# markvdw/GParML

Measured on AMD Instinct MI355X. Metric: variational bound+grad evals/sec, higher is better.
Workload: dtype f64

## Files before the change

gparml_amd/csrc/potrf128.h:

```cpp
#pragma once
#include <hip/hip_runtime.h>
#include "mma_f64.h"

#ifndef POTRF_STAMP
#define POTRF_STAMP(i)
#endif

namespace gp {

constexpr int NB = 128;

constexpr int PLD = NB + 2;

__device__ __forceinline__ void wave_sync() {
  asm volatile("s_waitcnt lgkmcnt(0)" ::: "memory");
  __builtin_amdgcn_wave_barrier();
}
__device__ __forceinline__ void block_sync_lds() {
  asm volatile("s_waitcnt lgkmcnt(0)" ::: "memory");
  __builtin_amdgcn_s_barrier();
  asm volatile("" ::: "memory");
}

__device__ __forceinline__ double readlane_f64(double v, int src) {
  const int lo = __builtin_amdgcn_readlane(__double2loint(v), src), hi = __builtin_amdgcn_readlane(__double2hiint(v), src);
  return __hiloint2double(hi, lo);
}

__device__ __forceinline__ double rsqrt_chain(double x) {
  const double y = __builtin_amdgcn_rsq(x);
  const double e = fma(-(x * y), y, 1.0);
  return fma(y * e, fma(e, 0.375, 0.5), y);
}

template <bool BT>
__device__ __forceinline__ void lds_mma16(const double* S, int ar, int ac, int br, int bc, int kb, int ke, int lane, double (&acc)[4]) {
  const int lr = lane & 15, lk = lane >> 4, lj = lane & 3;
  const double* pa = S + (ar + lr) * PLD + ac + lk;
  const double* pb = BT ? S + (br + lj) * PLD + bc + lk : S + (br + lk) * PLD + bc + lj;
  auto load = [&](int k0, double (&a)[4], double (&b)[4][4]) {
#pragma unroll
    for (int s = 0; s < 4; ++s) {
      const int k = k0 + 4 * s;
      a[s] = pa[k];
#pragma unroll
      for (int j = 0; j < 4; ++j) b[s][j] = BT ? pb[4 * j * PLD + k] : pb[k * PLD + 4 * j];
    }
  };
  auto mma = [&](const double (&a)[4], const double (&b)[4][4]) {
    __builtin_amdgcn_sched_barrier(0);
#pragma unroll
    for (int s = 0; s < 4; ++s)
#pragma unroll
      for (int j = 0; j < 4; ++j) acc[j] = __builtin_amdgcn_mfma_f64_4x4x4f64(a[s], b[s][j], acc[j], 0, 0, 0);
    __builtin_amdgcn_sched_barrier(0);
  };
  double a0[4], b0[4][4], a1[4], b1[4][4];
  if (kb < ke) load(kb, a0, b0);
  for (int k = kb; k < ke; k += 32) {
    const bool more1 = k + 16 < ke, more2 = k + 32 < ke;
    if (more1) load(k + 16, a1, b1);
    mma(a0, b0);
    if (more1) {
      if (more2) load(k + 32, a0, b0);
      mma(a1, b1);
    }
  }
}
__device__ __forceinline__ int t16_row(int lane) { return 4 * ((lane >> 2) & 3) + (lane >> 4); }
__device__ __forceinline__ int t16_col(int j, int lane) { return 4 * j + (lane & 3); }

constexpr int LSLD = 34;
constexpr int POTRF_LDS_DOUBLES = NB * PLD + 32 + 32 * LSLD + NB;

__global__ void __launch_bounds__(512) potrf_trinv128_kernel(double* A, long ld, long bstride, int j, double* Linv, double* fail,
                                                             double* logdet2) {
  extern __shared__ __attribute__((aligned(16))) double sm[];
  double* S = sm;
  double* Tw = S + NB * PLD;
  double* Lsp = Tw + 32;
  double* Dg = Lsp + 32 * LSLD;
  const int tid = threadIdx.x, lane = tid & 63, wave = __builtin_amdgcn_readfirstlane(tid >> 6);
  const long off = (long)blockIdx.x * bstride + ((long)j * NB) * ld + (long)j * NB;
  double* blk = A + off;
  double* xblk = Linv + off;
  {
    double2 v[16];
#pragma unroll
    for (int i = 0; i < 16; ++i) { const int e = tid + 512 * i; v[i] = *reinterpret_cast<const double2*>(blk + (long)(e >> 6) * ld + 2 * (e & 63)); }
#pragma unroll
    for (int i = 0; i < 16; ++i) {
      const int e = tid + 512 * i, r = e >> 6, c = 2 * (e & 63);
      *reinterpret_cast<double2*>(S + r * PLD + c) = make_double2(c <= r ? v[i].x : 0.0, c + 1 <= r ? v[i].y : 0.0);
    }
  }
  __syncthreads();
  POTRF_STAMP(0);
  double bad = 0.0;
  for (int s = 0; s < 4; ++s) {
    const int o = 32 * s;
    if (wave == 0) {
      const int i = lane & 31;
      double a[32];
#pragma unroll
      for (int p = 0; p < 16; ++p) {
        const double2 v = *reinterpret_cast<const double2*>(S + (o + i) * PLD + o + 2 * p);
        a[2 * p] = v.x; a[2 * p + 1] = v.y;
      }
      double myinv = 1.0, mydiag = 1.0;
      static_for<0, 32>([&](auto jc) {
        constexpr int j = decltype(jc)::value;
        const double d = readlane_f64(a[j], j);
        if (!(d > 0.0)) bad = fmax(bad, d == 0.0 ? 2.0 : 1.0);
        const double inv = rsqrt_chain(d);
        const double l = a[j] * inv;
        a[j] = l;
        if (i == j) { myinv = inv; mydiag = l; }
        static_for<j + 1, 32>([&](auto kc) {
          constexpr int k = decltype(kc)::value;
          a[k] = fma(-l, readlane_f64(l, k), a[k]);
        });
      });
      POTRF_STAMP(1 + 5 * s);
      if (lane < 32) {
#pragma unroll
        for (int p = 0; p < 16; ++p) {
          const double2 v = make_double2(2 * p <= i ? a[2 * p] : 0.0, 2 * p + 1 <= i ? a[2 * p + 1] : 0.0);
          *reinterpret_cast<double2*>(S + (o + i) * PLD + o + 2 * p) = v;
          *reinterpret_cast<double2*>(Lsp + i * LSLD + 2 * p) = v;
        }
        Tw[i] = myinv;
        Dg[o + i] = mydiag;
      }
      wave_sync();
      POTRF_STAMP(2 + 5 * s);
      if (lane < 32) {
        const int h = lane >> 4, cl = lane & 15;
        double w[16];
        double2 row[2][8];
        double dinv[2];
        const double* Ls = S + (o + 16 * h) * PLD + o + 16 * h;
        const double* Tl = Tw + 16 * h;
        auto load_row = [&](auto ic, double2 (&b)[8], double& d) {
          constexpr int i = decltype(ic)::value;
#pragma unroll
          for (int p = 0; p < (i + 1) / 2; ++p) b[p] = *reinterpret_cast<const double2*>(Ls + i * PLD + 2 * p);
          d = Tl[i];
        };
        load_row(IC<0>{}, row[0], dinv[0]);
        static_for<0, 16>([&](auto ic) {
          constexpr int i = decltype(ic)::value, cur = i & 1;
          if constexpr (i + 1 < 16) load_row(IC<i + 1>{}, row[cur ^ 1], dinv[cur ^ 1]);
          __builtin_amdgcn_sched_barrier(0);
          double s0 = (cl == i) ? 1.0 : 0.0, s1 = 0.0;
#pragma unroll
          for (int p = 0; p < i / 2; ++p) {
            s0 = fma(-row[cur][p].x, w[2 * p], s0);
            s1 = fma(-row[cur][p].y, w[2 * p + 1], s1);
          }
          if constexpr (i & 1) s0 = fma(-row[cur][i / 2].x, w[i - 1], s0);
          w[i] = (s0 + s1) * dinv[cur];
          __builtin_amdgcn_sched_barrier(0);
        });
#pragma unroll
        for (int i = 0; i < 16; ++i) S[(o + 16 * h + i) * PLD + o + 16 * h + cl] = w[i];
      }
      wave_sync();
      {
        double acc[4] = {0.0, 0.0, 0.0, 0.0};
        lds_mma16<false>(S, o + 16, o, o, o, 0, 16, lane, acc);
        wave_sync();
        const int R = o + 16 + t16_row(lane);
#pragma unroll
        for (int jj = 0; jj < 4; ++jj) { S[R * PLD + o + t16_col(jj, lane)] = acc[jj]; acc[jj] = 0.0; }
        wave_sync();
        lds_mma16<false>(S, o + 16, o + 16, o + 16, o, 0, 16, lane, acc);
        wave_sync();
#pragma unroll
        for (int jj = 0; jj < 4; ++jj) S[R * PLD + o + t16_col(jj, lane)] = -acc[jj];
      }
      wave_sync();
    }
    block_sync_lds();
    POTRF_STAMP(3 + 5 * s);
    if (wave == 7) {
#pragma unroll
      for (int it = 0; it < 8; ++it) {
        const int e = lane + 64 * it, r = e >> 4, c = 2 * (e & 15);
        *reinterpret_cast<double2*>(blk + (long)(o + r) * ld + o + c) = *reinterpret_cast<const double2*>(Lsp + r * LSLD + c);
      }
    }
    if (s == 3) break;
    const int nrb = (NB - o - 32) / 16;
    {
      double acc[2][4] = {{0.0, 0.0, 0.0, 0.0}, {0.0, 0.0, 0.0, 0.0}};
#pragma unroll
      for (int u = 0; u < 2; ++u) {
        const int t = wave + 8 * u;
        if (t < 2 * nrb) lds_mma16<true>(S, o + 32 + 16 * (t >> 1), o, o + 16 * (t & 1), o, 0, 16 * (t & 1) + 16, lane, acc[u]);
      }
      block_sync_lds();
#pragma unroll
      for (int u = 0; u < 2; ++u) {
        const int t = wave + 8 * u;
        if (t < 2 * nrb) {
          const int R = o + 32 + 16 * (t >> 1) + t16_row(lane);
#pragma unroll
          for (int jj = 0; jj < 4; ++jj) {
            const int C = o + 16 * (t & 1) + t16_col(jj, lane);
            S[R * PLD + C] = acc[u][jj];
            blk[(long)R * ld + C] = acc[u][jj];
          }
        }
      }
      block_sync_lds();
    }
    POTRF_STAMP(4 + 5 * s);
    auto update_tile = [&](int t) {
      int r16 = 0, rem = t;
      while (rem > r16) { rem -= r16 + 1; ++r16; }
      const int c16 = rem;
      double acc[4] = {0.0, 0.0, 0.0, 0.0};
      lds_mma16<true>(S, o + 32 + 16 * r16, o, o + 32 + 16 * c16, o, 0, 32, lane, acc);
      const int R = o + 32 + 16 * r16 + t16_row(lane);
#pragma unroll
      for (int jj = 0; jj < 4; ++jj) S[R * PLD + o + 32 + 16 * c16 + t16_col(jj, lane)] -= acc[jj];
    };
    const int ntile = nrb * (nrb + 1) / 2;
    if (wave < ntile) update_tile(wave);
    block_sync_lds();
    if (wave > 0)
      for (int t = 8 + (wave - 1); t < ntile; t += 7) update_tile(t);
    POTRF_STAMP(5 + 5 * s);
  }
  auto level = [&](auto bsc) {
    constexpr int bs = decltype(bsc)::value, tpp = (bs / 16) * (bs / 16), ntask = (NB / (2 * bs)) * tpp;
    double acc[2][4] = {{0.0, 0.0, 0.0, 0.0}, {0.0, 0.0, 0.0, 0.0}};
    int R0[2], C0[2], rb[2], cb[2];
#pragma unroll
    for (int u = 0; u < 2; ++u) {
      const int t = wave + 8 * u, p = t / tpp, tt = t % tpp;
      R0[u] = (2 * p + 1) * bs; C0[u] = 2 * p * bs; rb[u] = tt / (bs / 16); cb[u] = tt % (bs / 16);
      if (t < ntask) lds_mma16<false>(S, R0[u] + 16 * rb[u], C0[u], C0[u], C0[u] + 16 * cb[u], 16 * cb[u], bs, lane, acc[u]);
    }
    block_sync_lds();
#pragma unroll
    for (int u = 0; u < 2; ++u) {
      if (wave + 8 * u < ntask) {
        const int R = R0[u] + 16 * rb[u] + t16_row(lane);
#pragma unroll
        for (int jj = 0; jj < 4; ++jj) { S[R * PLD + C0[u] + 16 * cb[u] + t16_col(jj, lane)] = acc[u][jj]; acc[u][jj] = 0.0; }
      }
    }
    block_sync_lds();
#pragma unroll
    for (int u = 0; u < 2; ++u)
      if (wave + 8 * u < ntask) lds_mma16<false>(S, R0[u] + 16 * rb[u], R0[u], R0[u], C0[u] + 16 * cb[u], 0, 16 * rb[u] + 16, lane, acc[u]);
    block_sync_lds();
#pragma unroll
    for (int u = 0; u < 2; ++u) {
      if (wave + 8 * u < ntask) {
        const int R = R0[u] + 16 * rb[u] + t16_row(lane);
#pragma unroll
        for (int jj = 0; jj < 4; ++jj) S[R * PLD + C0[u] + 16 * cb[u] + t16_col(jj, lane)] = -acc[u][jj];
      }
    }
    block_sync_lds();
  };
  level(IC<32>{});
  level(IC<64>{});
  POTRF_STAMP(20);
  {
    int t2 = tid;
    asm volatile("" : "+v"(t2));
#pragma unroll
    for (int i = 0; i < 16; ++i) {
      const int e = t2 + 512 * i, r = e >> 6, c = 2 * (e & 63);
      const double2 x = *reinterpret_cast<const double2*>(S + r * PLD + c);
      *reinterpret_cast<double2*>(xblk + (long)r * ld + c) = make_double2(c <= r ? x.x : 0.0, c + 1 <= r ? x.y : 0.0);
      if (c > r) *reinterpret_cast<double2*>(blk + (long)r * ld + c) = make_double2(0.0, 0.0);
      else if (c == r) blk[(long)r * ld + c + 1] = 0.0;
    }
  }
  POTRF_STAMP(21);
  if (wave == 0) {
    double lg = log(Dg[lane]) + log(Dg[lane + 64]);
    for (int sh = 32; sh > 0; sh >>= 1) { lg += __shfl_xor(lg, sh); bad = fmax(bad, __shfl_xor(bad, sh)); }
    if (lane == 0) {
      if (bad != 0.0) fail[blockIdx.x] = fmax(fail[blockIdx.x], bad);
      logdet2[blockIdx.x] += 2.0 * lg;
    }
  }
}

}
```

Baseline: 57.48.

## Shrink Cholesky panel width to 16 and overlap diagonal factorization with trailing update

```diff
diff --git a/gparml_amd/csrc/potrf128.h b/gparml_amd/csrc/potrf128.h
--- a/gparml_amd/csrc/potrf128.h
+++ b/gparml_amd/csrc/potrf128.h
@@ -70,16 +70,17 @@
 __device__ __forceinline__ int t16_row(int lane) { return 4 * ((lane >> 2) & 3) + (lane >> 4); }
 __device__ __forceinline__ int t16_col(int j, int lane) { return 4 * j + (lane & 3); }
 
-constexpr int LSLD = 34;
-constexpr int POTRF_LDS_DOUBLES = NB * PLD + 32 + 32 * LSLD + NB;
+constexpr int SB = 16;
+constexpr int LSLD = 18;
+constexpr int POTRF_LDS_DOUBLES = NB * PLD + SB + 2 * SB * LSLD + NB;
 
 __global__ void __launch_bounds__(512) potrf_trinv128_kernel(double* A, long ld, long bstride, int j, double* Linv, double* fail,
                                                              double* logdet2) {
   extern __shared__ __attribute__((aligned(16))) double sm[];
   double* S = sm;
   double* Tw = S + NB * PLD;
-  double* Lsp = Tw + 32;
-  double* Dg = Lsp + 32 * LSLD;
+  double* Lsp = Tw + SB;
+  double* Dg = Lsp + 2 * SB * LSLD;
   const int tid = threadIdx.x, lane = tid & 63, wave = __builtin_amdgcn_readfirstlane(tid >> 6);
   const long off = (long)blockIdx.x * bstride + ((long)j * NB) * ld + (long)j * NB;
   double* blk = A + off;
@@ -97,18 +98,18 @@
   __syncthreads();
   POTRF_STAMP(0);
   double bad = 0.0;
-  for (int s = 0; s < 4; ++s) {
-    const int o = 32 * s;
+  for (int s = 0; s < NB / SB; ++s) {
+    const int o = SB * s;
     if (wave == 0) {
-      const int i = lane & 31;
-      double a[32];
-#pragma unroll
-      for (int p = 0; p < 16; ++p) {
+      const int i = lane & (SB - 1);
+      double a[SB];
+#pragma unroll
+      for (int p = 0; p < SB / 2; ++p) {
         const double2 v = *reinterpret_cast<const double2*>(S + (o + i) * PLD + o + 2 * p);
         a[2 * p] = v.x; a[2 * p + 1] = v.y;
       }
       double myinv = 1.0, mydiag = 1.0;
-      static_for<0, 32>([&](auto jc) {
+      static_for<0, SB>([&](auto jc) {
         constexpr int j = decltype(jc)::value;
         const double d = readlane_f64(a[j], j);
         if (!(d > 0.0)) bad = fmax(bad, d == 0.0 ? 2.0 : 1.0);
@@ -116,31 +117,31 @@
         const double l = a[j] * inv;
         a[j] = l;
         if (i == j) { myinv = inv; mydiag = l; }
-        static_for<j + 1, 32>([&](auto kc) {
+        static_for<j + 1, SB>([&](auto kc) {
           constexpr int k = decltype(kc)::value;
           a[k] = fma(-l, readlane_f64(l, k), a[k]);
         });
       });
-      POTRF_STAMP(1 + 5 * s);
-      if (lane < 32) {
-#pragma unroll
-        for (int p = 0; p < 16; ++p) {
+      POTRF_STAMP(1 + 4 * s);
+      double* Lcopy = Lsp + (s & 1) * SB * LSLD;
+      if (lane < SB) {
+#pragma unroll
+        for (int p = 0; p < SB / 2; ++p) {
           const double2 v = make_double2(2 * p <= i ? a[2 * p] : 0.0, 2 * p + 1 <= i ? a[2 * p + 1] : 0.0);
           *reinterpret_cast<double2*>(S + (o + i) * PLD + o + 2 * p) = v;
-          *reinterpret_cast<double2*>(Lsp + i * LSLD + 2 * p) = v;
+          *reinterpret_cast<double2*>(Lcopy + i * LSLD + 2 * p) = v;
         }
         Tw[i] = myinv;
         Dg[o + i] = mydiag;
       }
       wave_sync();
-      POTRF_STAMP(2 + 5 * s);
-      if (lane < 32) {
-        const int h = lane >> 4, cl = lane & 15;
+      if (lane < SB) {
+        const int cl = lane;
         double w[16];
         double2 row[2][8];
         double dinv[2];
-        const double* Ls = S + (o + 16 * h) * PLD + o + 16 * h;
-        const double* Tl = Tw + 16 * h;
+        const double* Ls = S + o * PLD + o;
+        const double* Tl = Tw;
         auto load_row = [&](auto ic, double2 (&b)[8], double& d) {
           constexpr int i = decltype(ic)::value;
 #pragma unroll
@@ -163,75 +164,54 @@
           __builtin_amdgcn_sched_barrier(0);
         });
 #pragma unroll
-        for (int i = 0; i < 16; ++i) S[(o + 16 * h + i) * PLD + o + 16 * h + cl] = w[i];
-      }
-      wave_sync();
-      {
-        double acc[4] = {0.0, 0.0, 0.0, 0.0};
-        lds_mma16<false>(S, o + 16, o, o, o, 0, 16, lane, acc);
-        wave_sync();
-        const int R = o + 16 + t16_row(lane);
-#pragma unroll
-        for (int jj = 0; jj < 4; ++jj) { S[R * PLD + o + t16_col(jj, lane)] = acc[jj]; acc[jj] = 0.0; }
-        wave_sync();
-        lds_mma16<false>(S, o + 16, o + 16, o + 16, o, 0, 16, lane, acc);
-        wave_sync();
-#pragma unroll
-        for (int jj = 0; jj < 4; ++jj) S[R * PLD + o + t16_col(jj, lane)] = -acc[jj];
-      }
-      wave_sync();
-    }
-    block_sync_lds();
-    POTRF_STAMP(3 + 5 * s);
+        for (int i = 0; i < 16; ++i) S[(o + i) * PLD + o + cl] = w[i];
+      }
+      wave_sync();
+      POTRF_STAMP(2 + 4 * s);
+    }
+    block_sync_lds();
     if (wave == 7) {
-#pragma unroll
-      for (int it = 0; it < 8; ++it) {
-        const int e = lane + 64 * it, r = e >> 4, c = 2 * (e & 15);
-        *reinterpret_cast<double2*>(blk + (long)(o + r) * ld + o + c) = *reinterpret_cast<const double2*>(Lsp + r * LSLD + c);
-      }
-    }
-    if (s == 3) break;
-    const int nrb = (NB - o - 32) / 16;
-    {
-      double acc[2][4] = {{0.0, 0.0, 0.0, 0.0}, {0.0, 0.0, 0.0, 0.0}};
-#pragma unroll
-      for (int u = 0; u < 2; ++u) {
-        const int t = wave + 8 * u;
-        if (t < 2 * nrb) lds_mma16<true>(S, o + 32 + 16 * (t >> 1), o, o + 16 * (t & 1), o, 0, 16 * (t & 1) + 16, lane, acc[u]);
-      }
-      block_sync_lds();
-#pragma unroll
-      for (int u = 0; u < 2; ++u) {
-        const int t = wave + 8 * u;
-        if (t < 2 * nrb) {
-          const int R = o + 32 + 16 * (t >> 1) + t16_row(lane);
-#pragma unroll
-          for (int jj = 0; jj < 4; ++jj) {
-            const int C = o + 16 * (t & 1) + t16_col(jj, lane);
-            S[R * PLD + C] = acc[u][jj];
-            blk[(long)R * ld + C] = acc[u][jj];
-          }
-        }
-      }
-      block_sync_lds();
-    }
-    POTRF_STAMP(4 + 5 * s);
+      const double* Lcopy = Lsp + (s & 1) * SB * LSLD;
+#pragma unroll
+      for (int it = 0; it < 2; ++it) {
+        const int e = lane + 64 * it, r = e >> 3, c = 2 * (e & 7);
+        *reinterpret_cast<double2*>(blk + (long)(o + r) * ld + o + c) = *reinterpret_cast<const double2*>(Lcopy + r * LSLD + c);
+      }
+    }
+    if (s == NB / SB - 1) break;
+    const int nrb = (NB - o - SB) / SB;
+    if (wave < nrb) {
+      double acc[4] = {0.0, 0.0, 0.0, 0.0};
+      lds_mma16<true>(S, o + SB + SB * wave, o, o, o, 0, SB, lane, acc);
+      wave_sync();
+      const int R = o + SB + SB * wave + t16_row(lane);
+#pragma unroll
+      for (int jj = 0; jj < 4; ++jj) {
+        const int C = o + t16_col(jj, lane);
+        S[R * PLD + C] = acc[jj];
+        blk[(long)R * ld + C] = acc[jj];
+      }
+    }
+    block_sync_lds();
+    POTRF_STAMP(3 + 4 * s);
     auto update_tile = [&](int t) {
       int r16 = 0, rem = t;
       while (rem > r16) { rem -= r16 + 1; ++r16; }
       const int c16 = rem;
       double acc[4] = {0.0, 0.0, 0.0, 0.0};
-      lds_mma16<true>(S, o + 32 + 16 * r16, o, o + 32 + 16 * c16, o, 0, 32, lane, acc);
-      const int R = o + 32 + 16 * r16 + t16_row(lane);
-#pragma unroll
-      for (int jj = 0; jj < 4; ++jj) S[R * PLD + o + 32 + 16 * c16 + t16_col(jj, lane)] -= acc[jj];
+      lds_mma16<true>(S, o + SB + SB * r16, o, o + SB + SB * c16, o, 0, SB, lane, acc);
+      const int R = o + SB + SB * r16 + t16_row(lane);
+#pragma unroll
+      for (int jj = 0; jj < 4; ++jj) S[R * PLD + o + SB + SB * c16 + t16_col(jj, lane)] -= acc[jj];
     };
     const int ntile = nrb * (nrb + 1) / 2;
-    if (wave < ntile) update_tile(wave);
-    block_sync_lds();
-    if (wave > 0)
-      for (int t = 8 + (wave - 1); t < ntile; t += 7) update_tile(t);
-    POTRF_STAMP(5 + 5 * s);
+    if (wave == 0) {
+      update_tile(0);
+      wave_sync();
+    } else {
+      for (int t = wave; t < ntile; t += 7) update_tile(t);
+    }
+    POTRF_STAMP(4 + 4 * s);
   }
   auto level = [&](auto bsc) {
     constexpr int bs = decltype(bsc)::value, tpp = (bs / 16) * (bs / 16), ntask = (NB / (2 * bs)) * tpp;
@@ -267,9 +247,10 @@
     }
     block_sync_lds();
   };
+  level(IC<16>{});
   level(IC<32>{});
   level(IC<64>{});
-  POTRF_STAMP(20);
+  POTRF_STAMP(33);
   {
     int t2 = tid;
     asm volatile("" : "+v"(t2));
@@ -282,7 +263,7 @@
       else if (c == r) blk[(long)r * ld + c + 1] = 0.0;
     }
   }
-  POTRF_STAMP(21);
+  POTRF_STAMP(34);
   if (wave == 0) {
     double lg = log(Dg[lane]) + log(Dg[lane + 64]);
     for (int sh = 32; sh > 0; sh >>= 1) { lg += __shfl_xor(lg, sh); bad = fmax(bad, __shfl_xor(bad, sh)); }
```

Result: no change. 57.69 (median of 6 runs) (+0.4%).
